# centreborelli/s2p

Hardware: NVIDIA H100
Metric: disparity_throughput_1024x1024x128_mgm (higher is better)
Workload: dtype f32

## Files before the change

### s2p_b200/csrc/agg_kernel.cuh

```cuda
#pragma once
#include <cuda_fp16.h>
#include <type_traits>
#include <cuda_runtime.h>
#include <stdint.h>

namespace s2pb {

#define S2PB_INF __int_as_float(0x7f800000)

constexpr int kMaxPasses = 8;
constexpr int kMaxPV = 16;
constexpr int kNW = 16;
constexpr int kNWC = 8;
constexpr int kAggThreads = kNWC * 32;
#ifndef S2PB_SYNC2
#define S2PB_SYNC2 1
#endif
#ifndef S2PB_SPLIT_LOOP
#define S2PB_SPLIT_LOOP 1
#endif
template <int LPL> struct SyncCfg {
    static constexpr bool sync2 = S2PB_SYNC2 && LPL > 4 && LPL <= 8;
    static constexpr int kRing = sync2 ? 8 : 4;
};
// ... 52 lines not shown
template <int LPL> __device__ __forceinline__ void ld_vec(const float *p, float (&v)[LPL])
{
    if constexpr (LPL % 4 == 0) {
#pragma unroll
        for (int q = 0; q < LPL / 4; q++) {
            float4 t = reinterpret_cast<const float4 *>(p)[q];
            v[4 * q] = t.x; v[4 * q + 1] = t.y; v[4 * q + 2] = t.z; v[4 * q + 3] = t.w;
        }
    } else if constexpr (LPL % 2 == 0) {
#pragma unroll
        for (int q = 0; q < LPL / 2; q++) {
            float2 t = reinterpret_cast<const float2 *>(p)[q];
            v[2 * q] = t.x; v[2 * q + 1] = t.y;
        }
    } else {
#pragma unroll
        for (int q = 0; q < LPL; q++) v[q] = p[q];
    }
}
template <int LPL> __device__ __forceinline__ void st_vec(float *p, const float (&v)[LPL])
{
    if constexpr (LPL % 4 == 0) {
#pragma unroll
        for (int q = 0; q < LPL / 4; q++)
            reinterpret_cast<float4 *>(p)[q] = make_float4(v[4 * q], v[4 * q + 1], v[4 * q + 2], v[4 * q + 3]);
    } else if constexpr (LPL % 2 == 0) {
#pragma unroll
        for (int q = 0; q < LPL / 2; q++) reinterpret_cast<float2 *>(p)[q] = make_float2(v[2 * q], v[2 * q + 1]);
    } else {
#pragma unroll
        for (int q = 0; q < LPL; q++) p[q] = v[q];
    }
}
#ifndef S2PB_STREAM_STORES
#define S2PB_STREAM_STORES 0
#endif
template <int LPL> __device__ __forceinline__ void st_vec_out(float *p, const float (&v)[LPL])
{
#if S2PB_STREAM_STORES
    if constexpr (LPL % 4 == 0) {
#pragma unroll
        for (int q = 0; q < LPL / 4; q++) __stcs(reinterpret_cast<float4 *>(p) + q, make_float4(v[4 * q], v[4 * q + 1], v[4 * q + 2], v[4 * q + 3]));
    } else if constexpr (LPL % 2 == 0) {
#pragma unroll
        for (int q = 0; q < LPL / 2; q++) __stcs(reinterpret_cast<float2 *>(p) + q, make_float2(v[2 * q], v[2 * q + 1]));
    } else {
#pragma unroll
        for (int q = 0; q < LPL; q++) __stcs(p + q, v[q]);
    }
#else
    st_vec<LPL>(p, v);
#endif
}
constexpr unsigned kCostInf = 0xFFu;
constexpr int kCostMaxCode = 127;
__host__ __device__ __forceinline__ unsigned cost_encode(unsigned cnt, bool finite) { return finite ? cnt : kCostInf; }
__device__ __forceinline__ unsigned char cost_encode_f(float c) { return isinf(c) ? (unsigned char)kCostInf : (unsigned char)(int)c; }
__device__ __forceinline__ float cost_decode(unsigned code) { return (code & 0x80u) ? S2PB_INF : (float)code; }
__device__ __forceinline__ unsigned prmt(unsigned a, unsigned b, unsigned sel)
{
    unsigned r;
    asm("prmt.b32 %0, %1, %2, %3;" : "=r"(r) : "r"(a), "r"(b), "r"(sel));
    return r;
}
template <int N> __device__ __forceinline__ void cost_decode_word(unsigned w, float *c)
{
    const __half2 k1024 = __half2half2(__ushort_as_half((unsigned short)0x6400));
#pragma unroll
    for (int j = 0; j < N; j += 2) {
        const unsigned h = prmt(w, 0x6464u, j == 0 ? 0x4140u : 0x4342u);
        const unsigned m = prmt(w, 0u, j == 0 ? 0x9988u : 0xbbaau);
        unsigned sel = (h & ~m) | (0x7c007c00u & m);
        const __half2 v = __hsub2(*reinterpret_cast<const __half2 *>(&sel), k1024);
        c[j] = __low2float(v);
        if (j + 1 < N) c[j + 1] = __high2float(v);
    }
}
template <int LPL> struct CostPack { unsigned w[(LPL + 3) / 4]; };
template <int LPL> __device__ __forceinline__ CostPack<LPL> cost_pack(const unsigned (&cnt)[LPL], unsigned fin)
{
    CostPack<LPL> r;
#pragma unroll
    for (int q = 0; q < (LPL + 3) / 4; q++) {
        unsigned v = 0;
#pragma unroll
// ... 50 lines not shown
        for (int q = 0; q < LPL / 16; q++) reinterpret_cast<uint4 *>(p)[q] = make_uint4(v.w[4 * q], v.w[4 * q + 1], v.w[4 * q + 2], v.w[4 * q + 3]);
    } else if constexpr (LPL % 8 == 0) {
#pragma unroll
        for (int q = 0; q < LPL / 8; q++) reinterpret_cast<uint2 *>(p)[q] = make_uint2(v.w[2 * q], v.w[2 * q + 1]);
    } else if constexpr (LPL % 4 == 0) {
#pragma unroll
        for (int q = 0; q < LPL / 4; q++) reinterpret_cast<unsigned *>(p)[q] = v.w[q];
    } else if constexpr (LPL % 2 == 0) {
#pragma unroll
        for (int q = 0; q < LPL / 2; q++) reinterpret_cast<unsigned short *>(p)[q] = (unsigned short)(v.w[q / 2] >> (16 * (q & 1)));
    } else {
#pragma unroll
        for (int q = 0; q < LPL; q++) p[q] = (uint8_t)(v.w[q / 4] >> (8 * (q & 3)));
    }
}
__device__ __forceinline__ float cost_scaled(float c, const float *__restrict__ lut)
{
    if (lut != nullptr && c >= 0.f && c < 64.f) c = lut[(int)c];
    return c;
}
__device__ __forceinline__ float cost_value(unsigned code, const float *__restrict__ lut) { return cost_scaled(cost_decode(code), lut); }


struct PassDesc {
    int nS, nI;
    long long base;
    int strideS, strideI;
    int type;
    int nBands;
    const void *C;
    const float *W;
    float *L;
    float *Lmin;
    int *progress;
};
struct AggParams {
    PassDesc pv[kMaxPV];
    int nPV, maxBands;
    float P1, P2;
    int *next_item;
    const int *abort_flag;
    const float *lut;
    int general;
};

template <int LPL, bool GEN = false> struct StageCfg {
#ifdef S2PB_STAGE
    static constexpr int kStage = GEN ? ((LPL <= 4) ? 8 : (LPL <= 8) ? 4 : 2) : ((LPL <= 12) ? S2PB_STAGE : 2);
#else
    static constexpr int kStage = GEN ? ((LPL <= 4) ? 8 : (LPL <= 8) ? 4 : 2) : ((LPL <= 12) ? 8 : 2);
#endif
    static constexpr int kR0 = 2 * kStage;
};

__device__ __forceinline__ void cp_async16(void *smem, const void *gmem)
{
    unsigned sa = (unsigned)__cvta_generic_to_shared(smem);
    asm volatile("cp.async.cg.shared.global [%0], [%1], 16;" ::"r"(sa), "l"(gmem) : "memory");
}
__device__ __forceinline__ void cp_async4(void *smem, const void *gmem)
{
    unsigned sa = (unsigned)__cvta_generic_to_shared(smem);
    asm volatile("cp.async.ca.shared.global [%0], [%1], 4;" ::"r"(sa), "l"(gmem) : "memory");
}
__device__ __forceinline__ void cp_async_commit() { asm volatile("cp.async.commit_group;" ::: "memory"); }
template <int N> __device__ __forceinline__ void cp_async_wait() { asm volatile("cp.async.wait_group %0;" ::"n"(N) : "memory"); }
// ... 143 lines not shown
                if (CH % 16 == 0 || q16 + 16 * q < CH) cp_async16_s(d + 256 * q, csrc + 256 * q);
            csrc += cstep;
            if (weighted) {
                if (q16 == 0) cp_async4_s(wdst + (unsigned)((jc & (kStage - 1)) * 4), wsrc);
                wsrc += strideI;
            }
        }
        jc++;
    };
    auto stage_prevband = [&]() {
        if (stage_prev) {
            if (jp < nI) {
                int spins = 0;
#ifndef S2PB_DIAG_NOPOLL
                while (avail < jp + 1) {
                    avail = ld_acquire(prev_progress);
                    if (((++spins) & 1023) == 0 && *(volatile const int *)abort_flag) break;
                }
#endif
                const unsigned slot = (unsigned)(jp & (kR0 - 1));
                warp_cp_async_s<DP * 4>(r0_s + slot * (DP * 4), psrc, lane);
                if (lane == 0) cp_async4_s(r0m_s + slot * 4, pmsrc);
                psrc += lstepb;
                pmsrc += strideI;
            }
            jp++;
        }
    };

    const long long lstep = strideI * DP;
    float *outA = pd.L + rowbaseA * DP + lane * LPL;
    float *outB = outA + (long long)pd.strideS * DP;
    float *lminB = pd.Lmin + rowbaseA + pd.strideS;

    auto fetch_prev = [&](int j, NbVec<LPL> &dst) {
        const int slot = j & srcmask;
        ld_vec<LPL>(srcring + slot * DP, dst.v);
        if (!MSG || from_r0) {
            dst.m = srcringm[slot];
            fill_edges<LPL>(dst, lane);
            if (MSG) nb_message<LPL>(dst, P1, P2);
        }
    };
    auto load_cost = [&](const CT *p, float (&c)[LPL]) {
        if constexpr (GEN) {
            ld_vec<LPL>(p, c);
        } else {
            cost_unpack<LPL>(ld_cost<LPL, false>(p), c);
            if (SCALED) {
#pragma unroll
                for (int e = 0; e < LPL; e++)
                    if (c[e] >= 0.f && c[e] < 64.f) c[e] = lut[(int)c[e]];
            }
        }
    };
    auto recurse2 = [&](const float (&cA)[LPL], const float (&cB)[LPL],
                        const NbVec<LPL> &aA, const NbVec<LPL> &aB, const NbVec<LPL> &aC, const NbVec<LPL> &aE,
                        const NbVec<LPL> &bA, const NbVec<LPL> &bB, const NbVec<LPL> &bC, const NbVec<LPL> &bE,
                        bool borderA, bool borderB, const float2 wv, float (&LA)[LPL], float (&LB)[LPL], auto interior_c) {
        constexpr bool INTERIOR = decltype(interior_c)::value;
        const float2 P1v = make_float2(P1, P1), P2v = make_float2(P2, P2);
        const float2 mA = make_float2(aA.m, bA.m), mB = make_float2(aB.m, bB.m), mC = make_float2(aC.m, bC.m), mE = make_float2(aE.m, bE.m);
        const float2 P1w = GEN ? make_float2(__fmul_rn(P1, wv.x), __fmul_rn(P1, wv.y)) : P1v;
        auto qof = [&](const float2 m) { return GEN ? fma2(P2v, wv, m) : add2(m, P2v); };
        const float2 qA = qof(mA), qB = qof(mB), qC = qof(mC), qE = qof(mE);
        const float2 nA = make_float2(-mA.x, -mA.y), nB = make_float2(-mB.x, -mB.y), nC = make_float2(-mC.x, -mC.y), nE = make_float2(-mE.x, -mE.y);
        constexpr int ordA = (TYPE == 0) ? 0 : 3, ordC = (TYPE == 0) ? 1 : 2, ordB = (TYPE == 0) ? 2 : 1, ordE = (TYPE == 0) ? 3 : 0;
        auto term = [&](const NbVec<LPL> &na, const NbVec<LPL> &nb, int e, const float2 q, const float2 negm, auto ord_c) {
            if constexpr (MSG) return make_float2(na.v[e], nb.v[e]);
            constexpr bool FMA1 = GEN && decltype(ord_c)::value >= 2;
            const float la = (e == 0) ? na.l : na.v[e - 1], ra = (e == LPL - 1) ? na.r : na.v[e + 1];
            const float lb = (e == 0) ? nb.l : nb.v[e - 1], rb = (e == LPL - 1) ? nb.r : nb.v[e + 1];
            const float2 mn = make_float2(fminf(la, ra), fminf(lb, rb));
            const float2 v1 = FMA1 ? fma2(P1v, wv, mn) : add2(mn, P1w);
// ... 53 lines not shown
        constexpr bool FAST = decltype(fast_c)::value;
        const int iA = t - k * WSK, iB = iA - SKEW;
        const bool actA = FAST || (liveA && iA >= 0 && iA < nI), actB = FAST || (liveB && iB >= 0 && iB < nI);
        NbVec<LPL> &inlineA = useE ? hE : hC;
        if (FAST || iA - rsel * SKEW >= 0) stage_cost();
        if (FAST || iA >= 0) stage_prevband();
        cp_async_commit();
        if (actA || actB) {
            cp_async_wait<S>();
            __syncwarp();
            float cA[LPL], cB[LPL], LA[LPL], LB[LPL];
#pragma unroll
            for (int e = 0; e < LPL; e++) cA[e] = cB[e] = 0.f;
            if (actA) load_cost(cstA + (iA & (kStage - 1)) * DP, cA);
            if (actB) load_cost(cstB + (iB & (kStage - 1)) * DP, cB);
            if (FAST) {
                if (useE) fetch_prev(iA + 1, xE); else fetch_prev(iA, xC);
            } else if (prevA && actA) {
                if (useE) { if (iA == 0) fetch_prev(0, xC); if (iA + 1 < nI) fetch_prev(iA + 1, xE); }
                else fetch_prev(iA, xC);
            }
            const bool borderA = (sA == 0) || (iA == 0) || (iA == nI - 1);
            const bool borderB = (iB == 0) || (iB == nI - 1);
            float2 wv = make_float2(1.f, 1.f);
            if (GEN) { if (weighted) { if (actA) wv.x = wstA[iA & (kStage - 1)]; if (actB) wv.y = wstB[iB & (kStage - 1)]; } }
            recurse2(cA, cB, inlineA, xB, xC, xE, wAB, hNew, hC, hE, borderA, borderB, wv, LA, LB, fast_c);
            const float mAm = vec_min(LA), mBm = vec_min(LB);
            if (actA) {
#pragma unroll
                for (int e = 0; e < LPL; e++) hNew.v[e] = LA[e];
                hNew.m = mAm;
                fill_edges<LPL>(hNew, lane);
                if (MSG) nb_message<LPL>(hNew, P1, P2);
                st_vec_out<LPL>(outA, LA);
                outA += lstep;
            }
            if (actB) {
#pragma unroll
                for (int e = 0; e < LPL; e++) wAB.v[e] = LB[e];
                wAB.m = mBm;
                if (MSG && (useA || usePrev)) {
                    fill_edges<LPL>(wAB, lane);
                    nb_message<LPL>(wAB, P1, P2);
                } else if (useA) {
                    fill_edges<LPL>(wAB, lane);
                }
                if (usePrev) st_vec<LPL>(myring + (iB & (kRing - 1)) * DP, MSG ? wAB.v : LB);
                st_vec_out<LPL>(outB, LB);
                outB += lstep;
                if (!MSG && lane == 0 && usePrev) myringm[iB & (kRing - 1)] = mBm;
                if (publish) {
                    if (lane == 0) *lminB = mBm;
                    lminB += strideI;
                    if (((iB + 1) % kPublish) == 0 || iB == nI - 1) {
                        __syncwarp();
                        if (lane == 0) st_release(pd.progress + band, iB + 1);
                    }
                }
            }
        }
#ifdef S2PB_DIAG_NOBAR
        __syncwarp();
#else
        if (!SYNC2 || (t & 1)) __syncthreads();
        else __syncwarp();
#endif
    };
    const bool can_fast = liveA && liveB && prevA;
    const int fast_lo = k * WSK + SKEW + 1, fast_hi = k * WSK + nI - 2;
    auto do_step = [&](const int t, NbVec<LPL> &xB, NbVec<LPL> &xC, NbVec<LPL> &xE, NbVec<LPL> &hNew, NbVec<LPL> &hC, NbVec<LPL> &hE) {
        if (can_fast && t >= fast_lo && t <= fast_hi) step(std::true_type{}, t, xB, xC, xE, hNew, hC, hE);
        else step(std::false_type{}, t, xB, xC, xE, hNew, hC, hE);
    };

#if S2PB_SPLIT_LOOP
    auto group = [&](auto fast_c, const int t) {
        if constexpr (U == 2) {
            step(fast_c, t, x1, x0, x2, h0, h1, h2);
            step(fast_c, t + 1, x0, x1, x2, h1, h0, h2);
        } else {
            step(fast_c, t, x1, x2, x0, h0, h1, h2);
// ... 60 lines not shown
```

### s2p_b200/csrc/mgm_kernels.cuh

```cuda
#pragma once
#include "agg_kernel.cuh"

namespace s2pb {


__global__ void census_kernel(const float *__restrict__ img, int w, int h, int r, uint64_t *__restrict__ codes)
{
    int x = blockIdx.x * blockDim.x + threadIdx.x, y = blockIdx.y * blockDim.y + threadIdx.y;
    if (x >= w || y >= h) return;
    float c = img[(size_t)y * w + x];
    uint64_t code = 0;
    for (int j = -r; j <= r; j++)
        for (int i = -r; i <= r; i++) {
            if (i == 0 && j == 0) continue;
            int xx = x + i, yy = y + j;
            unsigned bit = 0;
            if (xx >= 0 && xx < w && yy >= 0 && yy < h) bit = c < img[(size_t)yy * w + xx];
            code = (code << 1) | bit;
        }
    codes[(size_t)y * w + x] = code;
}

__global__ void prepare_view_kernel(const float *__restrict__ in, int n, int lo_all, int hi_all, int sentinel,
                                    float *__restrict__ clean, short *__restrict__ lo, short *__restrict__ hi)
// ... 339 lines not shown
        for (int e = ea; e <= eb; e++) {
            float c[1];
            if (cost_gen_labels<1>(P, p, x, y, l, hgh, P.gmin + 32 * e + lane, c)) anyfinite = true;
            dst[32 * e + lane] = c[0];
        }
        if (!__any_sync(0xffffffffu, anyfinite)) {
            for (int e = ea; e <= eb; e++) {
                const int o = P.gmin + 32 * e + lane;
                if (o >= l && o <= hgh) dst[32 * e + lane] = 0.f;
            }
        }
    }
}

__global__ void pack_cost_kernel(const float *__restrict__ Cin, size_t npix, int D, int DP, uint8_t *__restrict__ C)
{
    size_t i = (size_t)blockIdx.x * blockDim.x + threadIdx.x;
    if (i >= npix * DP) return;
    size_t p = i / DP; int k = (int)(i % DP);
    C[i] = cost_encode_f(k < D ? Cin[p * D + k] : S2PB_INF);
}
__global__ void unpack_cost_kernel(const uint8_t *__restrict__ C, size_t npix, int D, int DP, const float *__restrict__ lut,
                                   float *__restrict__ Cout)
{
    size_t i = (size_t)blockIdx.x * blockDim.x + threadIdx.x;
    if (i >= npix * D) return;
    size_t p = i / D; int k = (int)(i % D);
    Cout[i] = cost_value(C[p * DP + k], lut);
}


struct WtaParams {
    const float *L[kMaxPasses];
    const void *C;
    const short *lo, *hi;
    const float *lut;
    int ndir, gmin, fix_overcount, refine;
    float inv_zoom_div;
    size_t npix;
    float *S;
    int Dout;
    float *disp, *cost, *conf;
    float *pkr;
};

__device__ __forceinline__ float pkr_ratio(float secondmin, float firstmin)
{
    return (float)((double)secondmin / fmax((double)firstmin, 0.01));
}

__device__ __forceinline__ void vfit3(float v0, float v1, float v2, float &vmin, float &xmin)
{
    if ((v1 > v0) && (v1 > v2)) { vmin = v1; xmin = 0.f; return; }
    float slope = v2 - v1;
    if ((v2 - v1) < (v0 - v1)) slope = v0 - v1;
    xmin = __fdiv_rn(v0 - v2, 2.f * slope);
    vmin = fmaf(xmin - 1.f, slope, v2);
}
__device__ __forceinline__ void parabola3(float v0, float v1, float v2, float &vmin, float &xmin)
{
    if (v1 > v0 && v1 > v2) { xmin = 0.f; vmin = v1; return; }
    float c = v1;
    float b = __fdiv_rn(v2 - v0, 2.f);
    float a = __fdiv_rn(v2 - 2.f * v1 + v0, 2.f);
    float x = __fdiv_rn(-b, 2.f * a);
    if (x > 1.f) x = 1.f;
    if (x < -1.f) x = -1.f;
    vmin = fmaf(fmaf(a, x, b), x, c);
    xmin = x;
}


template <int LPL> struct WtaMap {
    static constexpr bool interleaved = (LPL == 3 || LPL == 5 || LPL == 6);
    static __device__ __forceinline__ int slot(int lane, int e) { return interleaved ? 32 * e + lane : lane * LPL + e; }
};
template <int LPL> __device__ __forceinline__ void wta_ld_pass(const float *px, int lane, float (&v)[LPL])
{
    if constexpr (WtaMap<LPL>::interleaved) {
#pragma unroll
        for (int e = 0; e < LPL; e++) v[e] = __ldcg(px + 32 * e + lane);
    } else ld_vec_cg<LPL>(px + lane * LPL, v);
}

template <int LPL> __device__ __forceinline__ int wta_add_pass(const float (&v)[LPL], int lane, float (&s)[LPL])
{
    float lm = v[0];
#pragma unroll
    for (int e = 1; e < LPL; e++) lm = fminf(lm, v[e]);
    const float md = warp_min_f32(lm);
    int a = -1;
#pragma unroll
    for (int e = 0; e < LPL; e++) { if (v[e] == md) a = WtaMap<LPL>::slot(lane, e); s[e] += v[e]; }
    return __reduce_max_sync(0xffffffffu, a);
}
template <int LPL>
__device__ __forceinline__ void wta_finish(const WtaParams &P, size_t p, int lane, float (&s)[LPL], const int (&am)[kMaxPasses],
                                           const float (&c)[LPL], float *sSrow, int plo, int phi)
{
    constexpr int DP = 32 * LPL;
    float best = S2PB_INF;
    int bidx = 0x7fffffff;
#pragma unroll
    for (int e = 0; e < LPL; e++) {
        if (P.fix_overcount == 1) s[e] = fmaf(-(float)(P.ndir - 1), c[e], s[e]);
        if (isfinite(s[e]) && best > s[e]) { best = s[e]; bidx = WtaMap<LPL>::slot(lane, e); }
    }
    const float m = warp_min_f32(best);
    int cand = (best == m && bidx != 0x7fffffff) ? bidx : 0x7fffffff;
    int kbest = __reduce_min_sync(0xffffffffu, cand);
    if (kbest > DP - 1) kbest = 0;
    const int o = P.gmin + kbest;
    float minP = (float)o, minL = m;

    int confi = 0;
#pragma unroll
    for (int d = 0; d < kMaxPasses; d++) confi += (am[d] == kbest) ? 1 : 0;

    if (P.S != nullptr || P.refine != 0) {
        __syncwarp();
#pragma unroll
        for (int e = 0; e < LPL; e++) sSrow[WtaMap<LPL>::slot(lane, e)] = s[e];
        __syncwarp();
    }
    if (P.S != nullptr) {
        const int lo = plo - P.gmin, hi = phi - P.gmin;
        for (int kk = lane; kk < P.Dout; kk += 32)
            P.S[p * P.Dout + kk] = (kk >= lo && kk <= hi) ? sSrow[kk] : S2PB_INF;
// ... 43 lines not shown
        for (int e = 0; e < LPL; e++) s[e] = 0.f;
        const int plo = __ldg(P.lo + p), phi = __ldg(P.hi + p);
        constexpr bool early_cost = !GEN && !WtaMap<LPL>::interleaved && LPL <= 8;
        CostPack<early_cost ? LPL : 1> cpk;
        if constexpr (early_cost) cpk = ld_cost<LPL, true>(reinterpret_cast<const uint8_t *>(P.C) + p * DP + lane * LPL);
#pragma unroll
        for (int g = 0; g < kMaxPasses; g += 4) {
            float v[4][LPL];
#pragma unroll
            for (int q = 0; q < 4; q++)
                if (g + q < ndir) wta_ld_pass<LPL>(P.L[g + q] + p * DP, lane, v[q]);
#pragma unroll
            for (int q = 0; q < 4; q++) {
                am[g + q] = -1;
                if (g + q < ndir) am[g + q] = wta_add_pass<LPL>(v[q], lane, s);
            }
        }
        float c[LPL];
        if constexpr (GEN) wta_ld_pass<LPL>(reinterpret_cast<const float *>(P.C) + p * DP, lane, c);
        else if constexpr (WtaMap<LPL>::interleaved) {
            const uint8_t *cp = reinterpret_cast<const uint8_t *>(P.C) + p * DP + lane;
#pragma unroll
            for (int e = 0; e < LPL; e++) c[e] = cost_value(__ldg(cp + 32 * e), P.lut);
        } else {
            CostPack<LPL> cp;
            if constexpr (early_cost) cp = cpk;
            else cp = ld_cost<LPL, true>(reinterpret_cast<const uint8_t *>(P.C) + p * DP + lane * LPL);
#pragma unroll
            for (int e = 0; e < LPL; e++) c[e] = cost_value(cost_code(cp, e), P.lut);
        }
        wta_finish<LPL>(P, p, lane, s, am, c, sSrow, plo, phi);
    }
}
template <int LPL, bool GEN>
__global__ void __launch_bounds__(kWtaThreads) __maxnreg__((LPL <= 4) ? 64 : 128) wta_kernel(const WtaParams P)
{
    __shared__ float sS[kWtaThreads / 32][32 * LPL];
    float *sSrow = sS[threadIdx.x >> 5];
    if (P.ndir == kMaxPasses) wta_pixels<LPL, GEN, kMaxPasses>(P, sSrow);
    else wta_pixels<LPL, GEN, 0>(P, sSrow);
}

template <bool GEN>
__global__ void __launch_bounds__(kWtaThreads) wta_chunked_kernel(const WtaParams P, int DP)
{
    extern __shared__ float sS_all[];
    const int lane = threadIdx.x & 31, wib = threadIdx.x >> 5;
    float *sS = sS_all + (size_t)wib * DP;
    size_t warp = ((size_t)blockIdx.x * blockDim.x + threadIdx.x) >> 5, nwarps = ((size_t)gridDim.x * blockDim.x) >> 5;
    for (size_t p = warp; p < P.npix; p += nwarps) {
        const int lo = P.lo[p] - P.gmin, hi = P.hi[p] - P.gmin;
        const int ea = lo >> 5, eb = hi >> 5;
        float pm[kMaxPasses];
        int pa[kMaxPasses];
#pragma unroll
        for (int d = 0; d < kMaxPasses; d++) { pm[d] = S2PB_INF; pa[d] = -1; }
        float best = S2PB_INF;
        int bidx = 0x7fffffff;
        for (int e = ea; e <= eb; e++) {
            const int kk = 32 * e + lane;
            float s = 0.f;
#pragma unroll
            for (int d = 0; d < kMaxPasses; d++)
                if (d < P.ndir) {
                    const float v = __ldcg(P.L[d] + p * DP + kk);
                    if (v < pm[d]) { pm[d] = v; pa[d] = kk; } else if (v == pm[d]) pa[d] = kk;
                    s += v;
                }
            const float c = GEN ? reinterpret_cast<const float *>(P.C)[p * DP + kk]
                                : cost_value(reinterpret_cast<const uint8_t *>(P.C)[p * DP + kk], P.lut);
            if (P.fix_overcount == 1) s = fmaf(-(float)(P.ndir - 1), c, s);
            if (isfinite(s) && best > s) { best = s; bidx = kk; }
            sS[kk] = s;
// ... 171 lines not shown
```

### s2p_b200/csrc/s2pb200.cu

```cuda
#include "../../include/s2pb200.h"
#include "mgm_kernels.cuh"
#include "multiscale_kernels.cuh"
#include "dct_kernels.cuh"
#include "homography_kernels.cuh"
#include "fusion_kernels.cuh"
#include "triangulation_kernels.cuh"
#include "pointcloud_kernels.cuh"
#include "sgbm_kernels.cuh"
#include "agg_dispatch.h"
#include "agg_chunked.cuh"

#include <algorithm>
#include <atomic>
#include <chrono>
#include <list>
#include <mutex>
#include <cmath>
#include <cstdarg>
#include <cstdio>
#include <cstring>
#include <cstdlib>
#include <string>
#include <thread>
#include <vector>
// ... 2 lines not shown


static thread_local std::string g_err;
static int fail(int code, const char *fmt, ...)
{
    char buf[512];
    va_list ap;
    va_start(ap, fmt);
    vsnprintf(buf, sizeof buf, fmt, ap);
    va_end(ap);
    g_err = buf;
    return code;
}
#define CK(call)                                                                                     \
    do {                                                                                             \
        cudaError_t e_ = (call);                                                                     \
        if (e_ != cudaSuccess)                                                                       \
            return fail(S2PB_ERR_CUDA, "%s failed: %s (%s:%d)", #call, cudaGetErrorString(e_), __FILE__, __LINE__); \
    } while (0)


struct ViewWS {
    float *img;
    float *rt;
    uint64_t *census_rt;
    int *rowlist;
    float *rowthr;
    RtState *rtstate;
    short *lo, *hi;
    uint64_t *census;
    void *C;
    float *L[kMaxPasses];
    float *Lmin[kMaxPasses];
    int *progress;
    float *disp, *cost, *conf, *tmp;
};
struct Slot {
    void *base = nullptr;
    size_t bytes = 0;
    int w = 0, h = 0, DP = 0, ndir = 0;
    int cbytes = 1;
    ViewWS v[2];
    int *next_item = nullptr;
    float *lut = nullptr;
    double *Ydct = nullptr;
    float *d_in[2] = {nullptr, nullptr};
    float *d_w[2] = {nullptr, nullptr};
    float *d_disp = nullptr, *d_conf = nullptr, *d_dispR = nullptr;
    uint8_t *d_mask = nullptr;
    char *io_base = nullptr;
    size_t io_pix = 0;
    float *h_in[2] = {nullptr, nullptr};
    float *h_disp = nullptr, *h_conf = nullptr, *h_dispR = nullptr;
    uint8_t *h_mask = nullptr;
    size_t h_pix = 0;
    char *arena = nullptr;
    size_t arena_cap = 0, arena_off = 0;
    int *d_small = nullptr;
    cudaStream_t stream = nullptr;
    cudaStream_t stream2 = nullptr;
    cudaEvent_t fork = nullptr, join = nullptr;
    cudaEvent_t ev[S2PB_T_COUNT + 1] = {};
    cudaEvent_t done = nullptr;
    bool timed = false;
    bool direct_out = false;
};
// ... 63 lines not shown
    size_t failed_ = 0;
};

static int lpl_for(int D)
{
    static const int opts[] = {1, 2, 3, 4, 5, 6, 8, 12, 16};
    for (int o : opts) if (32 * o >= D) return o;
    return -1;
}
static int max_bands(int w, int h) { return ((w > h ? w : h) + 1) / 2; }

static int slot_layout(Slot &s, int w, int h, int DP, int ndir, int cbytes, bool allocate)
{
    size_t npix = (size_t)w * h, off = 0;
    auto take = [&](size_t bytes) { size_t o = off; off = align_up(off + bytes, 256); return o; };
    char *b = (char *)s.base;
    int mb = max_bands(w, h);
    for (int vi = 0; vi < 2; vi++) {
        ViewWS &v = s.v[vi];
        size_t o;
        o = take(npix * 4); if (allocate) v.img = (float *)(b + o);
        o = take(npix * 2); if (allocate) v.lo = (short *)(b + o);
        o = take(npix * 2); if (allocate) v.hi = (short *)(b + o);
        o = take(npix * 8); if (allocate) v.census = (uint64_t *)(b + o);
        o = take(npix * 4); if (allocate) v.rt = (float *)(b + o);
        o = take(npix * 8); if (allocate) v.census_rt = (uint64_t *)(b + o);
        o = take(((size_t)h + w) * 4 + w + 16); if (allocate) v.rowlist = (int *)(b + o);
        o = take((size_t)h * 4); if (allocate) v.rowthr = (float *)(b + o);
        o = take(256); if (allocate) v.rtstate = (RtState *)(b + o);
        o = take(npix * DP * cbytes); if (allocate) v.C = (void *)(b + o);
        for (int p = 0; p < ndir; p++) {
            o = take(npix * DP * 4); if (allocate) v.L[p] = (float *)(b + o);
            o = take(npix * 4); if (allocate) v.Lmin[p] = (float *)(b + o);
        }
        o = take((size_t)kMaxPasses * mb * 4); if (allocate) v.progress = (int *)(b + o);
        o = take(npix * 4); if (allocate) v.disp = (float *)(b + o);
        o = take(npix * 4); if (allocate) v.cost = (float *)(b + o);
        o = take(npix * 4); if (allocate) v.conf = (float *)(b + o);
        o = take(npix * 4); if (allocate) v.tmp = (float *)(b + o);
    }
    size_t o;
    o = take(256); if (allocate) s.next_item = (int *)(b + o);
    o = take(256); if (allocate) s.lut = (float *)(b + o);
    o = take(npix * 8); if (allocate) s.Ydct = (double *)(b + o);
    if (!allocate) s.bytes = off;
    return 0;
}

static int slot_io_ensure(Slot &s, size_t npix)
{
    if (s.io_pix >= npix) return S2PB_OK;
    if (s.io_base) { CK(cudaStreamSynchronize(s.stream)); CK(cudaFree(s.io_base)); s.io_base = nullptr; s.io_pix = 0; }
    size_t stride = align_up(npix * 4, 256);
    cudaError_t e = cudaMalloc((void **)&s.io_base, stride * 8);
    if (e != cudaSuccess) { cudaGetLastError(); return fail(S2PB_ERR_NOMEM, "I/O staging of %zu bytes: %s", stride * 8, cudaGetErrorString(e)); }
    s.d_in[0] = (float *)s.io_base; s.d_in[1] = (float *)(s.io_base + stride);
    s.d_disp = (float *)(s.io_base + 2 * stride); s.d_conf = (float *)(s.io_base + 3 * stride);
    s.d_dispR = (float *)(s.io_base + 4 * stride); s.d_mask = (uint8_t *)(s.io_base + 5 * stride);
    s.d_w[0] = (float *)(s.io_base + 6 * stride); s.d_w[1] = (float *)(s.io_base + 7 * stride);
    s.io_pix = npix;
    return S2PB_OK;
}

static int slot_ensure(s2pb_ctx *ctx, Slot &s, int w, int h, int DP, int ndir, int cbytes = 1)
{
    Slot probe;
// ... 242 lines not shown
static int view_lpl(const int gminv[2], const int gmaxv[2], int vi) { return lpl_for(gmaxv[vi] - gminv[vi] + 1); }

static void fill_pass(PassDesc &pd, int pass, int w, int h)
{
    const long long W = w, H = h;
    switch (pass) {
    case 0: pd.nS = h; pd.nI = w; pd.base = 0;                     pd.strideS = w;  pd.strideI = 1;  pd.type = 0; break;
    case 1: pd.nS = h; pd.nI = w; pd.base = (H - 1) * W + (W - 1); pd.strideS = -w; pd.strideI = -1; pd.type = 0; break;
    case 2: pd.nS = w; pd.nI = h; pd.base = (H - 1) * W;           pd.strideS = 1;  pd.strideI = -w; pd.type = 0; break;
    case 3: pd.nS = w; pd.nI = h; pd.base = W - 1;                 pd.strideS = -1; pd.strideI = w;  pd.type = 0; break;
    case 4: pd.nS = h; pd.nI = w; pd.base = W - 1;                 pd.strideS = w;  pd.strideI = -1; pd.type = 1; break;
    case 5: pd.nS = w; pd.nI = h; pd.base = (H - 1) * W + (W - 1); pd.strideS = -1; pd.strideI = -w; pd.type = 1; break;
    case 6: pd.nS = h; pd.nI = w; pd.base = (H - 1) * W;           pd.strideS = -w; pd.strideI = 1;  pd.type = 1; break;
    default: pd.nS = w; pd.nI = h; pd.base = 0;                    pd.strideS = 1;  pd.strideI = w;  pd.type = 1; break;
    }
    pd.nBands = (pd.nS + kNW - 1) / kNW;
}

static bool wide_slab(int LPL) { return 32 * LPL > 512; }

static int launch_aggregate(s2pb_ctx *ctx, Slot &s, int nviews, int w, int h, int LPL, float P1, float P2, int ndir, int tsgm,
                            const float *lut, cudaStream_t st, bool general = false, const float *const *wgt = nullptr,
                            const int *gminv = nullptr, int first_view = 0, int ctas_per_sm = 0)
{
    AggParams P;
    memset(&P, 0, sizeof P);
    int mb = max_bands(w, h);
    P.nPV = 0; P.maxBands = 0;
    for (int vi = first_view; vi < first_view + nviews; vi++) {
        CK(cudaMemsetAsync(s.v[vi].progress, 0, (size_t)kMaxPasses * mb * 4, st));
        for (int p = 0; p < ndir; p++) {
            PassDesc &pd = P.pv[P.nPV++];
            fill_pass(pd, p, w, h);
            pd.C = s.v[vi].C; pd.L = s.v[vi].L[p]; pd.Lmin = s.v[vi].Lmin[p];
            pd.W = (general && wgt) ? wgt[vi] : nullptr;
            pd.progress = s.v[vi].progress + (size_t)p * mb;
            if (pd.nBands > P.maxBands) P.maxBands = pd.nBands;
        }
    }
    int *counter = s.next_item + 16 * first_view;
    P.P1 = P1; P.P2 = P2; P.next_item = counter; P.abort_flag = ctx->abort_flag; P.lut = general ? nullptr : lut;
    P.general = general ? 1 : 0;
    CK(cudaMemsetAsync(counter, 0, 4, st));
    if (wide_slab(LPL)) {
        ChunkedParams Q;
        memset(&Q, 0, sizeof Q);
        Q.A = P;
        Q.DP = 32 * LPL;
        int q = 0;
        for (int vi = first_view; vi < first_view + nviews; vi++)
            for (int p = 0; p < ndir; p++, q++) { Q.lo[q] = s.v[vi].lo; Q.hi[q] = s.v[vi].hi; Q.gmin[q] = gminv[vi]; }
        int rr = agg_chunked_launch(tsgm, Q, ctx->sm_count, st);
        if (rr == 0) { ctx->launches++; return S2PB_OK; }
        if (rr != -2) return fail(S2PB_ERR_CUDA, "chunked aggregation launch failed: %s", cudaGetErrorString(cudaGetLastError()));
    }
    int r = agg_launch(LPL, tsgm, P, ctx->sm_count, st, ctas_per_sm);
    if (r == -2) return fail(S2PB_ERR_UNSUPPORTED, "no aggregation kernel for %d labels per lane", LPL);
    if (r != 0) return fail(S2PB_ERR_CUDA, "aggregation launch failed: %s", cudaGetErrorString(cudaGetLastError()));
    ctx->launches++;
    return S2PB_OK;
}

static bool cost_strip_enabled() { static int v = -1; if (v < 0) { const char *e = getenv("S2PB_COST_STRIP"); v = e ? atoi(e) : 1; } return v != 0; }
template <int LPL> static void launch_cost_t(const uint64_t *cu, const uint64_t *cv, const uint64_t *cv1, int zoom, bool narrow, int w, int h,
                                             const short *lo, const short *hi, int gmin, uint8_t *C, int sm, cudaStream_t st)
{
    if constexpr (LPL <= 8) {
// ... 33 lines not shown
    LPL_SWITCH(LPL, launch_cost_t<K>(cu, cv, cv1, zoom, narrow, w, h, lo, hi, gmin, (uint8_t *)C, ctx->sm_count, st));
    CK(cudaGetLastError());
    ctx->launches++;
    return S2PB_OK;
}
static int launch_cost_gen(s2pb_ctx *ctx, int LPL, const CostGenParams &P, cudaStream_t st)
{
    LPL_SWITCH(LPL, launch_cost_gen_t<K>(P, ctx->sm_count, st));
    CK(cudaGetLastError());
    ctx->launches++;
    return S2PB_OK;
}
static int launch_wta(s2pb_ctx *ctx, int LPL, const WtaParams &P, cudaStream_t st, bool general = false)
{
    if (P.S == nullptr && wide_slab(LPL)) {
        const int DP = 32 * LPL;
        const size_t smem = (size_t)(kWtaThreads / 32) * DP * sizeof(float);
        if (general) wta_chunked_kernel<true><<<ctx->sm_count * 16, kWtaThreads, smem, st>>>(P, DP);
        else wta_chunked_kernel<false><<<ctx->sm_count * 16, kWtaThreads, smem, st>>>(P, DP);
        CK(cudaGetLastError());
        ctx->launches++;
        return S2PB_OK;
    }
    LPL_SWITCH(LPL, launch_wta_t<K>(P, ctx->sm_count, st, general));
    CK(cudaGetLastError());
    ctx->launches++;
    return S2PB_OK;
}

static void fill_wta(WtaParams &P, const ViewWS &v, int ndir, int gmin, const s2pb_mgm_params *p, const float *lut, size_t npix)
{
    memset(&P, 0, sizeof P);
    P.pkr = nullptr;
    for (int d = 0; d < ndir; d++) P.L[d] = v.L[d];
    P.C = v.C; P.lo = v.lo; P.hi = v.hi; P.lut = lut;
    P.ndir = ndir; P.gmin = gmin; P.fix_overcount = p->fix_overcount; P.refine = p->refine;
    P.inv_zoom_div = 1.f; P.npix = npix; P.S = nullptr; P.Dout = 0;
    P.disp = v.disp; P.cost = v.cost; P.conf = v.conf;
}


static int dct_tables(s2pb_ctx *ctx, int n, bool half, const s2pb_ctx::DctTab **out)
{
    if (n > 8192) return fail(S2PB_ERR_UNSUPPORTED, "tiles wider than 8192 px are not supported (DCT tables of %d x %d doubles)", n, n);
    std::lock_guard<std::mutex> lock(ctx->dct_mu);
    s2pb_ctx::DctTab *t = nullptr;
    for (auto &e : ctx->dct) if (e.n == n) t = &e;
    if (!t) { ctx->dct.push_back({n, nullptr, nullptr, nullptr, nullptr, nullptr}); t = &ctx->dct.back(); }
    const double pi = 3.14159265358979323846264338327950288;
    const size_t nn = (size_t)n * n;
    std::vector<double> h;
    auto upload = [&](double **dst, size_t count) -> int {
        cudaError_t e = cudaMalloc((void **)dst, count * sizeof(double));
        if (e != cudaSuccess) { cudaGetLastError(); *dst = nullptr; return fail(S2PB_ERR_NOMEM, "DCT table of %zu bytes: %s", count * 8, cudaGetErrorString(e)); }
        CK(cudaMemcpy(*dst, h.data(), count * sizeof(double), cudaMemcpyHostToDevice));
        return S2PB_OK;
    };
    int rc;
    if (!t->T10) {
        h.resize(nn);
        for (int k = 0; k < n; k++)
            for (int j = 0; j < n; j++) h[(size_t)k * n + j] = 2.0 * cos(pi * (j + 0.5) * k / n);
        if ((rc = upload(&t->T10, nn)) != S2PB_OK) return rc;
    }
    if (!t->T01) {
        h.resize(nn);
        for (int i = 0; i < n; i++)
// ... 1438 lines not shown
```

Baseline: 135.6.

## Store aggregated costs as split high/low halves and prune WTA loads

For LPL==4, the aggregation kernel now writes each aggregated cost vector as two planes of 16-bit halves: high halves first, then low halves. It also records a per-pass argmin index in a new Am buffer. The WTA kernel first reads only the high-half plane to bound each lane's sums from below and above. It then fetches the low halves only for lanes near a possible minimum, and reads the per-pass argmins from Am instead of recomputing them. This is meant to cut WTA memory traffic, at the price of extra argmin work and stores during aggregation, a more complex layout, and a change to how the r0 ring is read.

```diff
diff --git a/s2p_b200/csrc/agg_kernel.cuh b/s2p_b200/csrc/agg_kernel.cuh
--- a/s2p_b200/csrc/agg_kernel.cuh
+++ b/s2p_b200/csrc/agg_kernel.cuh
@@ -108,25 +108,64 @@
         for (int q = 0; q < LPL; q++) p[q] = v[q];
     }
 }
-#ifndef S2PB_STREAM_STORES
-#define S2PB_STREAM_STORES 0
-#endif
-template <int LPL> __device__ __forceinline__ void st_vec_out(float *p, const float (&v)[LPL])
-{
-#if S2PB_STREAM_STORES
+template <int LPL> struct HalfPack { unsigned w[(LPL + 1) / 2]; };
+template <int LPL> __device__ __forceinline__ unsigned half_of(const HalfPack<LPL> &p, int e) { return (p.w[e / 2] >> (16 * (e & 1))) & 0xffffu; }
+template <int LPL, bool CG> __device__ __forceinline__ HalfPack<LPL> ld_halves(const unsigned short *p)
+{
+    HalfPack<LPL> r;
     if constexpr (LPL % 4 == 0) {
 #pragma unroll
-        for (int q = 0; q < LPL / 4; q++) __stcs(reinterpret_cast<float4 *>(p) + q, make_float4(v[4 * q], v[4 * q + 1], v[4 * q + 2], v[4 * q + 3]));
+        for (int q = 0; q < LPL / 4; q++) {
+            const uint2 t = CG ? __ldcg(reinterpret_cast<const uint2 *>(p) + q) : reinterpret_cast<const uint2 *>(p)[q];
+            r.w[2 * q] = t.x; r.w[2 * q + 1] = t.y;
+        }
     } else if constexpr (LPL % 2 == 0) {
 #pragma unroll
-        for (int q = 0; q < LPL / 2; q++) __stcs(reinterpret_cast<float2 *>(p) + q, make_float2(v[2 * q], v[2 * q + 1]));
+        for (int q = 0; q < LPL / 2; q++) r.w[q] = CG ? __ldcg(reinterpret_cast<const unsigned *>(p) + q) : reinterpret_cast<const unsigned *>(p)[q];
     } else {
 #pragma unroll
-        for (int q = 0; q < LPL; q++) __stcs(p + q, v[q]);
-    }
-#else
-    st_vec<LPL>(p, v);
-#endif
+        for (int q = 0; q < (LPL + 1) / 2; q++) r.w[q] = 0;
+#pragma unroll
+        for (int e = 0; e < LPL; e++) r.w[e / 2] |= (unsigned)(CG ? __ldcg(p + e) : p[e]) << (16 * (e & 1));
+    }
+    return r;
+}
+template <int LPL> __device__ __forceinline__ void join_halves(const HalfPack<LPL> &hi, const HalfPack<LPL> &lo, float (&v)[LPL])
+{
+#pragma unroll
+    for (int e = 0; e < LPL; e++) v[e] = __uint_as_float((half_of<LPL>(hi, e) << 16) | half_of<LPL>(lo, e));
+}
+template <int LPL> __device__ __forceinline__ void st_halves(unsigned short *p, const float (&v)[LPL])
+{
+    HalfPack<LPL> hi, lo;
+#pragma unroll
+    for (int q = 0; q < (LPL + 1) / 2; q++) {
+        const unsigned a = __float_as_uint(v[2 * q]), b = (2 * q + 1 < LPL) ? __float_as_uint(v[2 * q + 1]) : 0u;
+        hi.w[q] = __byte_perm(a, b, 0x7632);
+        lo.w[q] = __byte_perm(a, b, 0x5410);
+    }
+    unsigned short *pl = p + 32 * LPL;
+    if constexpr (LPL % 4 == 0) {
+#pragma unroll
+        for (int q = 0; q < LPL / 4; q++) {
+            reinterpret_cast<uint2 *>(p)[q] = make_uint2(hi.w[2 * q], hi.w[2 * q + 1]);
+            reinterpret_cast<uint2 *>(pl)[q] = make_uint2(lo.w[2 * q], lo.w[2 * q + 1]);
+        }
+    } else if constexpr (LPL % 2 == 0) {
+#pragma unroll
+        for (int q = 0; q < LPL / 2; q++) { reinterpret_cast<unsigned *>(p)[q] = hi.w[q]; reinterpret_cast<unsigned *>(pl)[q] = lo.w[q]; }
+    } else {
+#pragma unroll
+        for (int e = 0; e < LPL; e++) { p[e] = (unsigned short)half_of<LPL>(hi, e); pl[e] = (unsigned short)half_of<LPL>(lo, e); }
+    }
+}
+template <int LPL> constexpr bool kHalves = (LPL == 4);
+template <int LPL> __device__ __forceinline__ int last_argmin(const float (&v)[LPL], float m, int lane)
+{
+    int a = -1;
+#pragma unroll
+    for (int e = 0; e < LPL; e++) if (v[e] == m) a = lane * LPL + e;
+    return __reduce_max_sync(0xffffffffu, a);
 }
 constexpr unsigned kCostInf = 0xFFu;
 constexpr int kCostMaxCode = 127;
@@ -243,6 +282,7 @@
     const float *W;
     float *L;
     float *Lmin;
+    unsigned short *Am;
     int *progress;
 };
 struct AggParams {
@@ -452,14 +492,24 @@
     float *outA = pd.L + rowbaseA * DP + lane * LPL;
     float *outB = outA + (long long)pd.strideS * DP;
     float *lminB = pd.Lmin + rowbaseA + pd.strideS;
+    const unsigned short *r0h = reinterpret_cast<const unsigned short *>(smem + SM::r0_off) + lane * LPL;
 
     auto fetch_prev = [&](int j, NbVec<LPL> &dst) {
         const int slot = j & srcmask;
-        ld_vec<LPL>(srcring + slot * DP, dst.v);
-        if (!MSG || from_r0) {
+        if (from_r0) {
+            if constexpr (kHalves<LPL>) {
+                const unsigned short *h = r0h + slot * 2 * DP;
+                join_halves<LPL>(ld_halves<LPL, false>(h), ld_halves<LPL, false>(h + DP), dst.v);
+            } else ld_vec<LPL>(srcring + slot * DP, dst.v);
             dst.m = srcringm[slot];
             fill_edges<LPL>(dst, lane);
             if (MSG) nb_message<LPL>(dst, P1, P2);
+        } else {
+            ld_vec<LPL>(srcring + slot * DP, dst.v);
+            if (!MSG) {
+                dst.m = srcringm[slot];
+                fill_edges<LPL>(dst, lane);
+            }
         }
     };
     auto load_cost = [&](const CT *p, float (&c)[LPL]) {
@@ -579,7 +629,11 @@
                 hNew.m = mAm;
                 fill_edges<LPL>(hNew, lane);
                 if (MSG) nb_message<LPL>(hNew, P1, P2);
-                st_vec_out<LPL>(outA, LA);
+                if constexpr (kHalves<LPL>) {
+                    st_halves<LPL>(reinterpret_cast<unsigned short *>(outA - lane * LPL) + lane * LPL, LA);
+                    const int a = last_argmin<LPL>(LA, mAm, lane);
+                    if (lane == 0) pd.Am[rowbaseA + iA * strideI] = (unsigned short)a;
+                } else st_vec<LPL>(outA, LA);
                 outA += lstep;
             }
             if (actB) {
@@ -593,7 +647,11 @@
                     fill_edges<LPL>(wAB, lane);
                 }
                 if (usePrev) st_vec<LPL>(myring + (iB & (kRing - 1)) * DP, MSG ? wAB.v : LB);
-                st_vec_out<LPL>(outB, LB);
+                if constexpr (kHalves<LPL>) {
+                    st_halves<LPL>(reinterpret_cast<unsigned short *>(outB - lane * LPL) + lane * LPL, LB);
+                    const int a = last_argmin<LPL>(LB, mBm, lane);
+                    if (lane == 0) pd.Am[rowbaseA + pd.strideS + iB * strideI] = (unsigned short)a;
+                } else st_vec<LPL>(outB, LB);
                 outB += lstep;
                 if (!MSG && lane == 0 && usePrev) myringm[iB & (kRing - 1)] = mBm;
                 if (publish) {
diff --git a/s2p_b200/csrc/mgm_kernels.cuh b/s2p_b200/csrc/mgm_kernels.cuh
--- a/s2p_b200/csrc/mgm_kernels.cuh
+++ b/s2p_b200/csrc/mgm_kernels.cuh
@@ -395,6 +395,7 @@
 
 struct WtaParams {
     const float *L[kMaxPasses];
+    const unsigned short *Am[kMaxPasses];
     const void *C;
     const short *lo, *hi;
     const float *lut;
@@ -457,6 +458,17 @@
     for (int e = 0; e < LPL; e++) { if (v[e] == md) a = WtaMap<LPL>::slot(lane, e); s[e] += v[e]; }
     return __reduce_max_sync(0xffffffffu, a);
 }
+template <int LPL> __device__ __forceinline__ HalfPack<LPL> wta_ld_halves(const unsigned short *px, int lane)
+{
+    if constexpr (WtaMap<LPL>::interleaved) {
+        HalfPack<LPL> r;
+#pragma unroll
+        for (int q = 0; q < (LPL + 1) / 2; q++) r.w[q] = 0;
+#pragma unroll
+        for (int e = 0; e < LPL; e++) r.w[e / 2] |= (unsigned)__ldcg(px + 32 * e + lane) << (16 * (e & 1));
+        return r;
+    } else return ld_halves<LPL, true>(px + lane * LPL);
+}
 template <int LPL>
 __device__ __forceinline__ void wta_finish(const WtaParams &P, size_t p, int lane, float (&s)[LPL], const int (&am)[kMaxPasses],
                                            const float (&c)[LPL], float *sSrow, int plo, int phi)
@@ -566,13 +578,110 @@
         wta_finish<LPL>(P, p, lane, s, am, c, sSrow, plo, phi);
     }
 }
+template <int LPL, bool GEN, int NDIR>
+__device__ __forceinline__ void wta_pixels_halves(const WtaParams &P, float *sSrow)
+{
+    constexpr int DP = 32 * LPL;
+    constexpr int kG = (LPL <= 8) ? 4 : 2;
+    const int ndir = NDIR ? NDIR : P.ndir;
+    const int lane = threadIdx.x & 31;
+    const bool full = GEN || P.S != nullptr || P.pkr != nullptr;
+    size_t warp = ((size_t)blockIdx.x * blockDim.x + threadIdx.x) >> 5, nwarps = ((size_t)gridDim.x * blockDim.x) >> 5;
+    for (size_t p = warp; p < P.npix; p += nwarps) {
+        const int plo = __ldg(P.lo + p), phi = __ldg(P.hi + p);
+        float c[LPL];
+        if constexpr (GEN) wta_ld_pass<LPL>(reinterpret_cast<const float *>(P.C) + p * DP, lane, c);
+        else if constexpr (WtaMap<LPL>::interleaved) {
+            const uint8_t *cp = reinterpret_cast<const uint8_t *>(P.C) + p * DP + lane;
+#pragma unroll
+            for (int e = 0; e < LPL; e++) c[e] = cost_value(__ldg(cp + 32 * e), P.lut);
+        } else {
+            const CostPack<LPL> cp = ld_cost<LPL, true>(reinterpret_cast<const uint8_t *>(P.C) + p * DP + lane * LPL);
+#pragma unroll
+            for (int e = 0; e < LPL; e++) c[e] = cost_value(cost_code(cp, e), P.lut);
+        }
+        bool load = true;
+        if (!full) {
+            const float ovc = -(float)(ndir - 1);
+            float slo[LPL], shi[LPL];
+#pragma unroll
+            for (int e = 0; e < LPL; e++) slo[e] = shi[e] = 0.f;
+#pragma unroll
+            for (int g = 0; g < kMaxPasses; g += kG) {
+                HalfPack<LPL> h[kG];
+#pragma unroll
+                for (int q = 0; q < kG; q++)
+                    if (g + q < ndir) h[q] = wta_ld_halves<LPL>(reinterpret_cast<const unsigned short *>(P.L[g + q]) + p * 2 * DP, lane);
+#pragma unroll
+                for (int q = 0; q < kG; q++)
+                    if (g + q < ndir) {
+#pragma unroll
+                        for (int e = 0; e < LPL; e++) {
+                            const unsigned u = half_of<LPL>(h[q], e) << 16;
+                            slo[e] = __fadd_rn(slo[e], __uint_as_float(u));
+                            shi[e] = __fadd_rn(shi[e], u == 0x7f800000u ? S2PB_INF : __uint_as_float(u | 0xffffu));
+                        }
+                    }
+            }
+            float mhi = S2PB_INF;
+#pragma unroll
+            for (int e = 0; e < LPL; e++) {
+                if (P.fix_overcount == 1) { slo[e] = fmaf(ovc, c[e], slo[e]); shi[e] = fmaf(ovc, c[e], shi[e]); }
+                if (isfinite(shi[e])) mhi = fminf(mhi, shi[e]);
+            }
+            mhi = warp_min_f32(mhi);
+            bool cand = false;
+#pragma unroll
+            for (int e = 0; e < LPL; e++) cand |= slo[e] <= mhi;
+            const unsigned b = __ballot_sync(0xffffffffu, cand);
+            const unsigned nb = b | (b << 1) | (b >> 31) | (b >> 1) | (b << 31);
+            load = (nb >> lane) & 1u;
+        }
+        float s[LPL];
+        if (load) {
+#pragma unroll
+            for (int e = 0; e < LPL; e++) s[e] = 0.f;
+#pragma unroll
+            for (int g = 0; g < kMaxPasses; g += kG) {
+                HalfPack<LPL> h[kG], l[kG];
+#pragma unroll
+                for (int q = 0; q < kG; q++)
+                    if (g + q < ndir) {
+                        const unsigned short *px = reinterpret_cast<const unsigned short *>(P.L[g + q]) + p * 2 * DP;
+                        h[q] = wta_ld_halves<LPL>(px, lane);
+                        l[q] = wta_ld_halves<LPL>(px + DP, lane);
+                    }
+#pragma unroll
+                for (int q = 0; q < kG; q++)
+                    if (g + q < ndir) {
+                        float v[LPL];
+                        join_halves<LPL>(h[q], l[q], v);
+#pragma unroll
+                        for (int e = 0; e < LPL; e++) s[e] += v[e];
+                    }
+            }
+        } else {
+#pragma unroll
+            for (int e = 0; e < LPL; e++) s[e] = S2PB_INF;
+        }
+        int am[kMaxPasses];
+#pragma unroll
+        for (int d = 0; d < kMaxPasses; d++) am[d] = (d < ndir) ? (int)__ldg(P.Am[d] + p) : -1;
+        wta_finish<LPL>(P, p, lane, s, am, c, sSrow, plo, phi);
+    }
+}
 template <int LPL, bool GEN>
 __global__ void __launch_bounds__(kWtaThreads) __maxnreg__((LPL <= 4) ? 64 : 128) wta_kernel(const WtaParams P)
 {
     __shared__ float sS[kWtaThreads / 32][32 * LPL];
     float *sSrow = sS[threadIdx.x >> 5];
-    if (P.ndir == kMaxPasses) wta_pixels<LPL, GEN, kMaxPasses>(P, sSrow);
-    else wta_pixels<LPL, GEN, 0>(P, sSrow);
+    if constexpr (kHalves<LPL>) {
+        if (P.ndir == kMaxPasses) wta_pixels_halves<LPL, GEN, kMaxPasses>(P, sSrow);
+        else wta_pixels_halves<LPL, GEN, 0>(P, sSrow);
+    } else {
+        if (P.ndir == kMaxPasses) wta_pixels<LPL, GEN, kMaxPasses>(P, sSrow);
+        else wta_pixels<LPL, GEN, 0>(P, sSrow);
+    }
 }
 
 template <bool GEN>
diff --git a/s2p_b200/csrc/s2pb200.cu b/s2p_b200/csrc/s2pb200.cu
--- a/s2p_b200/csrc/s2pb200.cu
+++ b/s2p_b200/csrc/s2pb200.cu
@@ -58,6 +58,7 @@
     void *C;
     float *L[kMaxPasses];
     float *Lmin[kMaxPasses];
+    unsigned short *Am[kMaxPasses];
     int *progress;
     float *disp, *cost, *conf, *tmp;
 };
@@ -187,6 +188,7 @@
         for (int p = 0; p < ndir; p++) {
             o = take(npix * DP * 4); if (allocate) v.L[p] = (float *)(b + o);
             o = take(npix * 4); if (allocate) v.Lmin[p] = (float *)(b + o);
+            o = take(npix * 2); if (allocate) v.Am[p] = (unsigned short *)(b + o);
         }
         o = take((size_t)kMaxPasses * mb * 4); if (allocate) v.progress = (int *)(b + o);
         o = take(npix * 4); if (allocate) v.disp = (float *)(b + o);
@@ -495,7 +497,7 @@
         for (int p = 0; p < ndir; p++) {
             PassDesc &pd = P.pv[P.nPV++];
             fill_pass(pd, p, w, h);
-            pd.C = s.v[vi].C; pd.L = s.v[vi].L[p]; pd.Lmin = s.v[vi].Lmin[p];
+            pd.C = s.v[vi].C; pd.L = s.v[vi].L[p]; pd.Lmin = s.v[vi].Lmin[p]; pd.Am = s.v[vi].Am[p];
             pd.W = (general && wgt) ? wgt[vi] : nullptr;
             pd.progress = s.v[vi].progress + (size_t)p * mb;
             if (pd.nBands > P.maxBands) P.maxBands = pd.nBands;
@@ -595,7 +597,7 @@
 {
     memset(&P, 0, sizeof P);
     P.pkr = nullptr;
-    for (int d = 0; d < ndir; d++) P.L[d] = v.L[d];
+    for (int d = 0; d < ndir; d++) { P.L[d] = v.L[d]; P.Am[d] = v.Am[d]; }
     P.C = v.C; P.lo = v.lo; P.hi = v.hi; P.lut = lut;
     P.ndir = ndir; P.gmin = gmin; P.fix_overcount = p->fix_overcount; P.refine = p->refine;
     P.inv_zoom_div = 1.f; P.npix = npix; P.S = nullptr; P.Dout = 0;
```

Measured after the change: 137.7 (median of 6 runs). 1.02x the previous value.
